# kofinandi/pixel-nerf-yolo

Hardware: NVIDIA B200
Metric: rays/sec (samples/sec) 3-view render at 1/2/4/8 B200 vs host-CPU ref (higher is better)
Workload: dtype bf16

## Files before the change

### pixel-nerf-yolo_b200/csrc/mlp_umma_pair.cu

```cuda
#include "pnr_common.cuh"
#include "umma.cuh"
#include <cuda.h>
#include <stdlib.h>
#include <vector>

namespace pnr {
using namespace umma;

namespace pair {

#ifdef PNR_DIAG_MMAONLY
#define PNR_DIAG_OFF_RING
#define PNR_DIAG_OFF_WAITS
#define PNR_DIAG_OFF_EPI
#define PNR_DIAG_OFF_GATHER
#endif
#ifdef PNR_DIAG_NORING
#define PNR_DIAG_OFF_RING
#define PNR_DIAG_OFF_EMPTY_COMMIT
#endif

constexpr int kNCol = 64;
constexpr int kMT = 2;
constexpr int kKBlocksH = kHidden / kBlockK;
#ifndef PNR_STAGES
#define PNR_STAGES 5
#endif
constexpr int kStages = PNR_STAGES;
constexpr int kThreads = 512;
constexpr int kProducers = 3;
constexpr int kGatherWarps = 4;
constexpr int kEpiWarps = 8;
constexpr int kOperandKB = kNCol * kRowBytes;
constexpr int kChunkBytes = 2 * kOperandKB;
constexpr int kTmemCols = 512;
constexpr int kHCol = 256;
constexpr int kMaxStages = 1024;

struct Sched { int n_blocks, CL, n_linz, KBz, order, proj; };
enum { MAT_LIN_IN = 0, MAT_LINZ = 1, MAT_FC0 = 2, MAT_FC1 = 3, MAT_LIN_OUT = 4 };
struct Seg { int kind, blk, t, len; };
struct StageSrc { int mat, blk, row0, k0; };

__host__ __device__ inline int z_passes(const Sched& s) { return (s.KBz + 7) / 8; }
__host__ __device__ inline int sched_total(const Sched& s) {
  return kMT + s.n_linz * kMT * s.KBz + s.n_blocks * 32 + kKBlocksH;
}
__host__ __device__ inline int sched_pre(const Sched& s) { return kMT + s.n_linz * kMT * s.KBz + s.CL * 32; }
__host__ __device__ inline void fc_pair(int order, int t, int& kc, int& mt, int& kk, bool& first, bool& last) {
  const int pr = t >> 1;
  kk = t & 1;
  if (order == 0) {
    kc = pr >> 1; mt = pr & 1;
    first = pr < 2 && kk == 0; last = pr >= 6 && kk == 1;
    return;
  }
  if (order == 3) {
    kc = (int)((0x23023101u >> (4 * pr)) & 0xFu);
    mt = (int)((0xE4u >> pr) & 1u);
    first = (pr == 0 || pr == 2) && kk == 0;
    last = (pr == 4 || pr == 7) && kk == 1;
    return;
  }
  kc = (pr < 4) ? (pr & 1) : (2 + (pr & 1));
  if (order == 2) kc ^= 1;
  mt = (pr >> 1) & 1;
  first = (pr == 0 || pr == 2) && kk == 0;
  last = (pr == 5 || pr == 7) && kk == 1;
}
__host__ __device__ inline int out_chunk(int order, int t) { return order >= 2 ? ((t >> 1) ^ 1) : (t >> 1); }
__host__ __device__ inline Seg walk_stage(const Sched& sc, int s) {
  Seg g;
  const int s1 = kMT * sc.KBz;
  if (s < kMT) { g.kind = MAT_LIN_IN; g.blk = 0; g.t = s; g.len = kMT; return g; }
  s -= kMT;
  if (s < s1) { g.kind = MAT_LINZ; g.blk = 0; g.t = s; g.len = s1; return g; }
  s -= s1;
  for (int b = 0; b < sc.n_blocks; ++b) {
    const bool has_z = b + 1 < sc.n_linz;
    if (s < 16) { g.kind = MAT_FC0; g.blk = b; g.t = s; g.len = 16; return g; }
    s -= 16;
    if (has_z) {
      if (s < s1) { g.kind = MAT_LINZ; g.blk = b + 1; g.t = s; g.len = s1; return g; }
      s -= s1;
    }
    if (s < 16) { g.kind = MAT_FC1; g.blk = b; g.t = s; g.len = 16; return g; }
    s -= 16;
  }
  g.kind = MAT_LIN_OUT; g.blk = 0; g.t = s; g.len = kKBlocksH;
  return g;
}
struct ZPos { int pass, mt, kbi, kp; };
__host__ __device__ inline ZPos z_position(int KBz, int t) {
  ZPos z;
  z.pass = t / (kMT * 8);
  const int tt = t - z.pass * kMT * 8;
  z.kp = KBz - z.pass * 8 < 8 ? KBz - z.pass * 8 : 8;
  z.mt = tt / z.kp;
  z.kbi = tt - z.mt * z.kp;
  return z;
}
__host__ __device__ inline StageSrc decode_stage(const Sched& sc, int s) {
  const Seg g = walk_stage(sc, s);
  StageSrc r;
  r.mat = g.kind; r.blk = g.blk;
  switch (g.kind) {
    case MAT_LIN_IN: r.row0 = g.t * 256; r.k0 = 0; break;
    case MAT_LINZ: { const ZPos z = z_position(sc.KBz, g.t); r.row0 = z.mt * 256; r.k0 = (z.pass * 8 + z.kbi) * 64; } break;
    case MAT_FC0:
    case MAT_FC1: { int kc, mt, kk; bool f, l; fc_pair(sc.order, g.t, kc, mt, kk, f, l); r.row0 = mt * 256; r.k0 = kc * 128 + kk * 64; } break;
    default: r.row0 = 0; r.k0 = out_chunk(sc.order, g.t) * 128 + (g.t & 1) * 64; break;
  }
  return r;
}

__global__ void pack_stages_kernel(pnr_mlp_params mp, Sched sc, uint8_t* __restrict__ stages) {
  const int s = blockIdx.x >> 1, half = blockIdx.x & 1;
  const StageSrc src = decode_stage(sc, s);
  const float* W; int rows, cols;
  switch (src.mat) {
    case MAT_LIN_IN: W = mp.lin_in_w; rows = mp.d_hidden; cols = mp.d_in; break;
    case MAT_LINZ: W = mp.linz_w[src.blk]; rows = mp.d_hidden; cols = mp.d_latent; break;
    case MAT_FC0: W = mp.fc0_w[src.blk]; rows = mp.d_hidden; cols = mp.d_hidden; break;
    case MAT_FC1: W = mp.fc1_w[src.blk]; rows = mp.d_hidden; cols = mp.d_hidden; break;
    default: W = mp.lin_out_w; rows = mp.d_out; cols = mp.d_hidden; break;
  }
  const bool identity = sc.proj && src.mat == MAT_LINZ;
  uint8_t* dst = stages + ((size_t)s * 2 + half) * kStageBytes;
  for (int i = threadIdx.x; i < kStageRows * kBlockK; i += blockDim.x) {
    const int r = i / kBlockK, k = i % kBlockK;
    const int gr = src.row0 + half * 128 + r, gk = src.k0 + k;
    const float v = identity ? (gr == gk ? 1.f : 0.f) : ((gr < rows && gk < cols) ? W[(size_t)gr * cols + gk] : 0.f);
    *reinterpret_cast<__nv_bfloat16*>(dst + swz_offset(r, k)) = __float2bfloat16_rn(v);
  }
}

struct Smem {
  static constexpr uint32_t w = 0;
  static constexpr uint32_t ring = w + kStages * kStageBytes;
  static constexpr uint32_t lat = ring + 4 * kChunkBytes;
  static constexpr uint32_t zf = lat + kKBlocksH * kOperandKB;
  static constexpr uint32_t bars = zf + kOperandKB;
  static constexpr uint32_t prog = bars + 512;
  static constexpr uint32_t total = prog + 8 * kMaxStages;
};
enum {
  B_W_FULL = 0, B_W_EMPTY = B_W_FULL + kStages, B_IN_READY = B_W_EMPTY + kStages, B_IN_FREE,
  B_X_FULL, B_H_FULL = B_X_FULL + kMT,
  B_RDY = B_H_FULL + kMT, B_X_FREE = B_RDY + 4,
  B_LAND = B_X_FREE + kMT,
  B_OUT_FREE = B_LAND + kMT,
  B_C0_FREE,
  B_COUNT
};
static_assert(B_COUNT <= 30, "barrier parity bits live in one 32-bit word");
static_assert(Smem::total <= 227 * 1024, "shared memory budget");

struct ProgEntry { uint32_t w0, w1; };
__device__ inline ProgEntry make_prog(const Sched& sc, int s, uint32_t sbase) {
  const Seg g = walk_stage(sc, s);
  uint32_t b_addr = 0, dcol = 0, acc = 1, wait_id = 0, c1 = 0, c2 = 0, c3 = 0;
  const bool last = g.t == g.len - 1;
  switch (g.kind) {
    case MAT_LIN_IN:
      b_addr = sbase + Smem::zf; dcol = g.t * 128; acc = 0;
      if (g.t == 0) wait_id = B_IN_READY + 1;
      break;
    case MAT_LINZ: {
      const ZPos z = z_position(sc.KBz, g.t);
      const bool streaming = z_passes(sc) > 1 || sc.proj;
      const bool pass_first = z.mt == 0 && z.kbi == 0, pass_last = z.mt == kMT - 1 && z.kbi == z.kp - 1;
      b_addr = sbase + Smem::lat + z.kbi * kOperandKB; dcol = z.mt * 128;
      if (streaming && pass_first && !(g.blk == 0 && z.pass == 0)) wait_id = B_IN_READY + 1;
      if (pass_last && (streaming || g.blk == sc.n_linz - 1)) c1 = B_IN_FREE + 1;
      if (last && g.blk == 0) { c2 = B_X_FULL + 1; c3 = B_X_FULL + 2; }
    } break;
    case MAT_FC0:
    case MAT_FC1: {
      int kc, mt, kk;
      bool first_of_tile, last_of_tile;
      fc_pair(sc.order, g.t, kc, mt, kk, first_of_tile, last_of_tile);
      const bool fc0 = g.kind == MAT_FC0;
      b_addr = sbase + Smem::ring + (kc * 2 + kk) * kOperandKB; dcol = (fc0 ? kHCol : 0) + mt * 128;
      if (fc0) acc = first_of_tile ? 0 : 1;
      if (mt == 0 && kk == 0) wait_id = B_RDY + kc + 1;
      if (last_of_tile) c2 = (fc0 ? B_H_FULL : B_X_FULL) + mt + 1;
      if (sc.order == 3 && g.t == 11) c1 = B_C0_FREE + 1;
    } break;
    default: {
      const int kc = out_chunk(sc.order, g.t), kk = g.t % 2;
      b_addr = sbase + Smem::ring + (kc * 2 + kk) * kOperandKB; dcol = kHCol; acc = g.t > 0;
      if (kk == 0) wait_id = B_RDY + kc + 1;
      if (last) c2 = B_H_FULL + 1;
    } break;
  }
  ProgEntry e;
  e.w0 = ((b_addr >> 4) & 0x3FFFu) | (dcol << 14) | (acc << 23) | (wait_id << 25);
  e.w1 = c1 | (c2 << 5) | (c3 << 14) | ((c1 | c2 | c3) ? (1u << 19) : 0u);
  return e;
}

__device__ __forceinline__ int gather_col(int gw, int i) { return gw + kGatherWarps * i; }

__device__ __forceinline__ uint32_t pack_relu_bf16x2(float lo, float hi) {
  uint32_t d;
  asm("cvt.rn.relu.bf16x2.f32 %0, %1, %2;" : "=r"(d) : "f"(hi), "f"(lo));
  return d;
}

template <int NC, bool REMOTE, bool ADD_BIAS>
__device__ __forceinline__ void store_transposed(uint32_t base, const uint32_t* vals, float bias, int lane, int kq, int row0,
                                                 uint32_t async_bar = 0) {
  const int g = lane >> 3, i = lane & 7;
  const int k = kq + 8 * g;
  const uint32_t kb_off = (uint32_t)(k >> 6) * kOperandKB;
#pragma unroll
  for (int c0 = 0; c0 < NC; c0 += 16) {
    uint32_t p[8];
#ifdef PNR_DIAG_EPI_NOALU
#pragma unroll
    for (int j = 0; j < 8; ++j) p[j] = (uint32_t)(lane + j + c0);
#else
#pragma unroll
    for (int j = 0; j < 8; ++j) {
      float x = __uint_as_float(vals[c0 + j]), y = __uint_as_float(vals[c0 + 8 + j]);
      if (ADD_BIAS) { x += bias; y += bias; }
      p[j] = pack_relu_bf16x2(x, y);
    }
    transpose8x8(p, lane);
#endif
    const uint32_t e0 = __byte_perm(p[0], p[1], 0x5410), e1 = __byte_perm(p[2], p[3], 0x5410);
// ... 32 lines not shown
  const int pair_id = blockIdx.x >> 1, n_pairs = gridDim.x >> 1;
  constexpr int PP = kNCol / NS;
  constexpr int G = kNCol / PP;
  constexpr int NLIVE = G * PP;
  const bool pooled = NS > 1 || sch.CL < sch.n_blocks;
  const int n_sg = ((n_tiles + 1) / 2 + G - 1) / G;
  float* const xbar = xbar_all + (size_t)pair_id * (2 * kNCol * kHidden);
  extern __shared__ __align__(1024) uint8_t smem[];
  const uint32_t sbase = smem_u32(smem);
  volatile uint32_t* tmem_base_slot = reinterpret_cast<volatile uint32_t*>(smem + Smem::bars + 8 * B_COUNT);
  const int warp = __shfl_sync(0xffffffffu, (int)(threadIdx.x >> 5), 0);
  const int lane = threadIdx.x & 31;
  long long* const prof = (PROF == 1 && g_prof_pair) ? reinterpret_cast<long long*>(smem + Smem::bars + 256) : nullptr;
  if (prof && threadIdx.x < 32) prof[threadIdx.x] = 0;
  long long* const trace = (PROF == 2 && g_trace_pair && (blockIdx.x >> 1) == 0) ? g_trace_pair : nullptr;
  int n_tr = 0;
  const bool trace_stages = PROF == 2 && trace && g_trace_stages;
  auto bar = [&](int i) -> uint32_t { return sbase + Smem::bars + 8u * i; };
  auto lbar = [&](int i) -> uint32_t { return mapa_u32(sbase + Smem::bars + 8u * i, 0); };
  if ((sbase & 1023u) != 0) { if (threadIdx.x == 0) printf("pnr: dynamic smem not 1024-aligned\n"); __trap(); }

  if (threadIdx.x == 0) {
    for (int i = 0; i < kStages; ++i) { mbar_init(bar(B_W_FULL + i), 1); mbar_init(bar(B_W_EMPTY + i), 1); }
    mbar_init(bar(B_IN_READY), 2 * kGatherWarps);
    mbar_init(bar(B_IN_FREE), 1);
    for (int i = 0; i < kMT; ++i) { mbar_init(bar(B_X_FULL + i), 1); mbar_init(bar(B_H_FULL + i), 1); }
    for (int i = 0; i < 4; ++i) mbar_init(bar(B_RDY + i), kEpiWarps + ((ASYNC && (i & 1) == 0) ? 1 : 0));
    for (int i = 0; i < kMT; ++i) mbar_init(bar(B_LAND + i), kEpiWarps);
    mbar_init(bar(B_OUT_FREE), 2);
    mbar_init(bar(B_C0_FREE), 1);
    for (int i = 0; i < kMT; ++i) mbar_init(bar(B_X_FREE + i), 2 * kEpiWarps);
    fence_barrier_init();
  }
  const int n_stages = sched_total(sch);
  const int s_pre = sched_pre(sch);
  const int n_flat = G * s_pre + (n_stages - s_pre);
  for (int i = threadIdx.x; i < n_stages; i += kThreads) {
    const ProgEntry pe = make_prog(sch, i, sbase);
    reinterpret_cast<ProgEntry*>(smem + Smem::prog)[i] = pe;
    if (i == n_stages - 1) reinterpret_cast<ProgEntry*>(smem + Smem::prog)[n_stages] = pe;
  }
  if (warp == 1) tmem_alloc_2sm(sbase + Smem::bars + 8 * B_COUNT, kTmemCols);
  tc_fence_before();
  __syncthreads();
  cluster_sync_all();
  tc_fence_after();
  const uint32_t tmem_base = __shfl_sync(0xffffffffu, *tmem_base_slot, 0);
  if (warp == 4) PTRACE_L0(1 + (int)crank, 0xFF);
#ifdef PNR_DIAG_N
  const uint32_t idesc = instr_desc_bf16_2sm(PNR_DIAG_N);
#else
  const uint32_t idesc = instr_desc_bf16_2sm(2 * kNCol);
#endif

  if (warp == 0 || warp == 12 || warp == 13) {
    const int pid = warp == 0 ? 0 : warp - 11;
    if (elect_one()) {
      uint32_t slot = pid, par = 1;
      int carry = pid;
      for (int sg = pair_id; sg < n_sg; sg += n_pairs) {
        int fi = carry;
        int st = fi < G * s_pre ? fi % s_pre : fi - (G - 1) * s_pre;
        for (; fi < n_flat; fi += kProducers) {
#ifdef PNR_DIAG_OFF_RING
          continue;
#endif
          PTRACE(5 + pid + 3 * (int)crank, 0x10 + B_W_EMPTY + slot);
#if PNR_IDLE_WAIT
          mbar_wait_idle(bar(B_W_EMPTY + slot), par);
#else
          mbar_wait_cluster(bar(B_W_EMPTY + slot), par);
#endif
          PTRACE(5 + pid + 3 * (int)crank, 0x40 + B_W_EMPTY + slot);
#ifdef PNR_DIAG_NOWEIGHTS
          if (crank == 0) mbar_arrive(bar(B_W_FULL + slot));
#else
          if (crank == 0) mbar_arrive_expect_tx(bar(B_W_FULL + slot), 2 * kStageBytes);
          tma_load_2d_2sm(sbase + Smem::w + slot * kStageBytes, &wmap, 0, (st * 2 + (int)crank) * kStageRows, bar(B_W_FULL + slot));
#endif
          PTRACE(5 + pid + 3 * (int)crank, 0x84);
          slot += kProducers;
          if (slot >= kStages) { slot -= kStages; par ^= 1; }
          const int nf = fi + kProducers;
          if (nf < G * s_pre) { st += kProducers; if (st >= s_pre) st -= s_pre; }
          else st = nf - (G - 1) * s_pre;
        }
        carry = fi - n_flat;
      }
    }
    __syncwarp();
  } else if (warp == 1) {
    if (crank == 0) {
      const long long t_role0 = prof ? clock64() : 0;
      if (elect_one()) {
        uint32_t slot = 0, wpar = 0, ph = 0;
        uint32_t full_bar = bar(B_W_FULL), empty_bar = bar(B_W_EMPTY);
        const uint64_t wdesc0 = smem_desc(sbase + Smem::w);
        uint64_t a_desc = wdesc0;
        const uint64_t bdesc_hi = smem_desc(0);
        constexpr uint64_t kStageStep = kStageBytes >> 4;
        const uint2* prog = reinterpret_cast<const uint2*>(smem + Smem::prog);
#define MPROF_T0() const long long t0__ = prof ? clock64() : 0
#define MPROF_ADD(slot_) do { if (prof) prof[slot_] += clock64() - t0__; } while (0)
        for (int sg = pair_id; sg < n_sg; sg += n_pairs) {
          for (int seg = 0; seg <= G; ++seg) {
            const bool after_mean = seg > 0 && seg < G;
            if (after_mean) {
              MPROF_T0();
#ifndef PNR_DIAG_OFF_WAITS
              mbar_wait_cluster(bar(B_X_FREE), (ph >> B_X_FREE) & 1u);
#endif
              ph ^= (1u << B_X_FREE);
              tc_fence_after();
              MPROF_ADD(5);
            }
            const int st_beg = seg < G ? 0 : s_pre, st_end = seg < G ? s_pre : n_stages;
            if (seg == 0 && sg != pair_id) {
#ifndef PNR_DIAG_OFF_WAITS
              mbar_wait(bar(B_OUT_FREE), (ph >> B_OUT_FREE) & 1u);
#endif
              ph ^= (1u << B_OUT_FREE);
            }
            uint2 cur = prog[st_beg];
            auto issue_stage = [&](int st) {
              const uint2 nxt = prog[st + 1];
              const uint32_t wait_id = cur.x >> 25;
              if (wait_id) {
                MPROF_T0();
                const uint32_t id = wait_id - 1;
                PTRACE(0, 0x10 + id);
#ifndef PNR_DIAG_OFF_WAITS
                mbar_wait_cluster(bar(id), (ph >> id) & 1u);
#endif
                ph ^= (1u << id);
                PTRACE(0, 0x40 + id);
                if (ASYNC) fence_proxy_async();
                tc_fence_after();
                MPROF_ADD(id == B_IN_READY ? 2 : 4);
              }
#ifndef PNR_DIAG_OFF_RING
              {
                MPROF_T0();
                mbar_wait(full_bar, wpar);
                MPROF_ADD(1);
                if (trace_stages) PTRACE(0, 0x72);
              }
#endif
              const uint64_t b_desc = bdesc_hi | (uint64_t)(cur.x & 0x3FFFu);
              const uint32_t d_col = (cur.x >> 14) & 0x1FFu;
              mma_kblock_desc_2sm(tmem_base + d_col, a_desc, b_desc, idesc, (cur.x >> 23) & 1u);
#ifndef PNR_DIAG_OFF_EMPTY_COMMIT
              mma_commit_2sm(empty_bar, 3);
#endif
              if (cur.y & (1u << 19)) {
                const uint32_t c1 = cur.y & 31u, c2 = (cur.y >> 5) & 31u, c3 = (cur.y >> 14) & 31u;
                if (c1) mma_commit_2sm(bar(c1 - 1), 3);
                if (c2) mma_commit_2sm(bar(c2 - 1), 3);
                if (c3) mma_commit_2sm(bar(c3 - 1), 3);
                if (PROF == 2 && c2 > B_X_FULL && c2 <= B_X_FULL + 4) PTRACE(0, c2 - B_X_FULL);
              }
              if (trace_stages) PTRACE(0, 0x71);
              if (++slot == kStages) { slot = 0; wpar ^= 1; full_bar = bar(B_W_FULL); empty_bar = bar(B_W_EMPTY); a_desc = wdesc0; }
              else { full_bar += 8; empty_bar += 8; a_desc += kStageStep; }
              cur = nxt;
            };
            int st = st_beg;
            if (after_mean) {
              issue_stage(st++);
              MPROF_T0();
#ifndef PNR_DIAG_OFF_WAITS
              mbar_wait_cluster(bar(B_X_FREE + 1), (ph >> (B_X_FREE + 1)) & 1u);
#endif
              ph ^= (1u << (B_X_FREE + 1));
              tc_fence_after();
              MPROF_ADD(5);
            }
            for (; st < st_end; ++st) issue_stage(st);
          }
        }
#undef MPROF_T0
#undef MPROF_ADD
      }
      __syncwarp();
      if (prof && lane == 0) prof[0] += clock64() - t_role0;
#ifdef PNR_DIAG_OFF_EPI
    } else if (false) {
#else
    } else if (ASYNC) {
#endif
      const int n_pub = G * 2 * sch.CL + 2 * (sch.n_blocks - sch.CL) + 1;
      uint32_t par = 0;
      for (int sg = pair_id; sg < n_sg; sg += n_pairs) {
        for (int i = 0; i < n_pub; ++i) {
#pragma unroll
          for (int mt = 0; mt < kMT; ++mt) {
            mbar_wait_cluster(bar(B_LAND + mt), par);
// ... 273 lines not shown
              const uint4* src = reinterpret_cast<const uint4*>(fl0 + vb + off);
              r[2 * k] = __ldg(src); r[2 * k + 1] = __ldg(src + 1);
            } else {
              r[2 * k] = make_uint4(0u, 0u, 0u, 0u); r[2 * k + 1] = make_uint4(0u, 0u, 0u, 0u);
            }
          }
        };
        auto blend_col = [&](int i, const uint4 (&r)[8], const float (&w)[4]) {
          if (!act) return;
          float acc[16];
#pragma unroll
          for (int j = 0; j < 16; ++j) acc[j] = 0.f;
#pragma unroll
          for (int k = 0; k < 4; ++k) {
            const __nv_bfloat162* h0 = reinterpret_cast<const __nv_bfloat162*>(&r[2 * k]);
            const __nv_bfloat162* h1 = reinterpret_cast<const __nv_bfloat162*>(&r[2 * k + 1]);
#pragma unroll
            for (int j = 0; j < 4; ++j) {
              const float2 f0 = __bfloat1622float2(h0[j]), f1 = __bfloat1622float2(h1[j]);
              acc[2 * j] += w[k] * f0.x; acc[2 * j + 1] += w[k] * f0.y;
              acc[8 + 2 * j] += w[k] * f1.x; acc[8 + 2 * j + 1] += w[k] * f1.y;
            }
          }
          uint4 o0, o1;
          __nv_bfloat162* q0 = reinterpret_cast<__nv_bfloat162*>(&o0);
          __nv_bfloat162* q1 = reinterpret_cast<__nv_bfloat162*>(&o1);
#pragma unroll
          for (int j = 0; j < 4; ++j) {
            q0[j] = __floats2bfloat162_rn(acc[2 * j], acc[2 * j + 1]);
            q1[j] = __floats2bfloat162_rn(acc[8 + 2 * j], acc[8 + 2 * j + 1]);
          }
          const int c = gather_col(gw, i);
          uint8_t* kb_base = smem + Smem::lat + (lane >> 2) * kOperandKB;
          const int k_in = (lane & 3) * 16;
          *reinterpret_cast<uint4*>(kb_base + swz_offset(c, k_in)) = o0;
          *reinterpret_cast<uint4*>(kb_base + swz_offset(c, k_in + 8)) = o1;
        };
        {
          uint4 ra[8], rb[8];
          float wa[4], wb[4];
          load_col(0, ra, wa);
          load_col(1, rb, wb);
          {
            PPROF_T0();
            if (gw == 0 && crank == 0) PTRACE_L0(4, 0x10 + B_IN_FREE);
#if PNR_IDLE_WAIT
            mbar_wait_idle(bar(B_IN_FREE), par_free);
#else
            mbar_wait_cluster(bar(B_IN_FREE), par_free);
#endif
            if (gw == 0 && crank == 0) PTRACE_L0(4, 0x40 + B_IN_FREE);
            if (gw == 0) PPROF_ADD(17);
          }
          par_free ^= 1;
          if (fill == 0) {
#pragma unroll 1
            for (int i = 0; i < 16; ++i) zfeat_col(i);
          }
#pragma unroll 1
          for (int i = 0; i < 16; i += 2) {
            blend_col(i, ra, wa);
            if (i + 2 < 16) load_col(i + 2, ra, wa);
            blend_col(i + 1, rb, wb);
            if (i + 3 < 16) load_col(i + 3, rb, wb);
          }
        }
        fence_proxy_async();
        __syncwarp();
        if (lane == 0) { if (crank == 0) mbar_arrive(bar(B_IN_READY)); else mbar_arrive_cluster_relaxed(lbar(B_IN_READY)); }
        if (gw == 0 && crank == 0) PTRACE_L0(4, 0x83);
      }
    }
    if (prof && gw == 0 && lane == 0) prof[16] += clock64() - t_role0;
  }

  tc_fence_before();
  __syncthreads();
  if (PROF == 1 && g_prof_pair && threadIdx.x < 32) g_prof_pair[(size_t)blockIdx.x * 32 + threadIdx.x] = prof[threadIdx.x];
  cluster_sync_all();
  if (warp == 1) tmem_dealloc_2sm(tmem_base, kTmemCols);
}

}

static bool pair_async() {
  static int cached = -1;
  if (cached < 0) { const char* e = getenv("PNR_ASYNC"); cached = (e && atoi(e) == 0) ? 0 : 1; }
  return cached != 0;
}
static int pair_order() {
  static int cached = -1;
  if (cached < 0) { const char* e = getenv("PNR_ORDER"); cached = e ? atoi(e) : 2; if (cached < 0 || cached > 3) cached = 2; }
  return cached;
}
static pair::Sched pair_sched(const pnr_mlp_params* p, int proj) {
  return pair::Sched{p->n_blocks, p->combine_layer, p->combine_layer, proj ? kHidden / 64 : p->d_latent / 64, pair_order(), proj};
}
size_t pair_stream_bytes(const pnr_mlp_params* p, int proj) {
  pair::Sched s = pair_sched(p, proj);
  return (size_t)pair::sched_total(s) * 2 * kStageBytes;
}
int pair_stages(const pnr_mlp_params* p, int proj) {
  pair::Sched s = pair_sched(p, proj);
  return pair::sched_total(s);
}
int pair_pack(const pnr_mlp_params* p, uint8_t* stream, int proj, cudaStream_t st) {
  pair::Sched s = pair_sched(p, proj);
  PNR_REQUIRE(pair::sched_total(s) < pair::kMaxStages, PNR_ERR_UNSUPPORTED, "pair_pack: %d stages exceed the stage program (one padding entry is needed)", pair::sched_total(s));
  pair::pack_stages_kernel<<<pair::sched_total(s) * 2, 256, 0, st>>>(*p, s, stream);
  PNR_CHECK_LAUNCH("pair::pack_stages_kernel");
  return PNR_OK;
}

size_t pair_workspace_bytes() {
  int dev = 0, sms = 148;
  cudaGetDevice(&dev);
  cudaDeviceGetAttribute(&sms, cudaDevAttrMultiProcessorCount, dev);
  return (size_t)(sms / 2) * 2 * pair::kNCol * kHidden * sizeof(float);
}

int field_forward_pair(const pnr_scene* sc, const pnr_points* q, const pnr_mlp_params* mp, const uint8_t* stream,
                       const float* bx, const float* bh, const float* bo, float* out, void* ws, size_t ws_bytes,
                       int num_freqs, float freq_factor, int raw, int proj, cudaStream_t st) {
  PNR_REQUIRE(ws && ws_bytes >= pair_workspace_bytes() && ((uintptr_t)ws & 15) == 0, PNR_ERR_ARG,
              "field_forward_pair: workspace of pnr_field_workspace_bytes() = %zu bytes required (got %zu)",
              pair_workspace_bytes(), ws_bytes);
  float* xbar = (float*)ws;
  pair::Sched sch = pair_sched(mp, proj);
  const int PP = pair::kNCol / sc->NS;
  const int tiles_per_obj = (q->P + PP - 1) / PP;
  const long long n_tiles_ll = (long long)tiles_per_obj * sc->SB;
  PNR_REQUIRE(n_tiles_ll < (1LL << 31), PNR_ERR_ARG, "field_forward_pair: too many tiles");
  const int n_tiles = (int)n_tiles_ll;
  typedef CUresult (*EncodeFn)(CUtensorMap*, CUtensorMapDataType, cuuint32_t, void*, const cuuint64_t*, const cuuint64_t*,
                               const cuuint32_t*, const cuuint32_t*, CUtensorMapInterleave, CUtensorMapSwizzle,
                               CUtensorMapL2promotion, CUtensorMapFloatOOBfill);
  static EncodeFn encode = nullptr;
  if (!encode) {
    void* fn = nullptr;
    cudaDriverEntryPointQueryResult qres;
    cudaError_t e = cudaGetDriverEntryPoint("cuTensorMapEncodeTiled", &fn, cudaEnableDefault, &qres);
    PNR_REQUIRE(e == cudaSuccess && fn, PNR_ERR_CUDA, "cuTensorMapEncodeTiled entry point not found");
    encode = (EncodeFn)fn;
  }
  CUtensorMap tmap;
  cuuint64_t gdim[2] = {64, (cuuint64_t)pair::sched_total(sch) * 256};
  cuuint64_t gstride[1] = {128};
  cuuint32_t box[2] = {64, 128};
  cuuint32_t estr[2] = {1, 1};
  CUresult r = encode(&tmap, CU_TENSOR_MAP_DATA_TYPE_BFLOAT16, 2, (void*)stream, gdim, gstride, box, estr,
                      CU_TENSOR_MAP_INTERLEAVE_NONE, CU_TENSOR_MAP_SWIZZLE_NONE, CU_TENSOR_MAP_L2_PROMOTION_L2_256B,
                      CU_TENSOR_MAP_FLOAT_OOB_FILL_NONE);
  PNR_REQUIRE(r == CUDA_SUCCESS, PNR_ERR_CUDA, "cuTensorMapEncodeTiled failed (%d)", (int)r);
  int dev = 0, sms = 148;
  cudaGetDevice(&dev);
  cudaDeviceGetAttribute(&sms, cudaDevAttrMultiProcessorCount, dev);
  const int G = pair::kNCol / PP;
  const bool async_x = pair_async();
  const bool vmax = mp->combine_type == PNR_COMBINE_MAX && sc->NS > 1;
  PNR_REQUIRE(!vmax || (async_x && !getenv("PNR_TRACE") && !getenv("PNR_PROF")), PNR_ERR_UNSUPPORTED,
              "field_forward_pair: the PNR_ASYNC=0 / PNR_PROF / PNR_TRACE instruments are built for combine_type average only");
  const int n_groups = ((n_tiles + 1) / 2 + G - 1) / G;
  long long* prof_dev = nullptr;
  long long* trace_dev = nullptr;
  if (getenv("PNR_TRACE")) {
    cudaMalloc(&trace_dev, (size_t)11 * pair::kTraceLen * sizeof(long long));
    cudaMemset(trace_dev, 0, (size_t)11 * pair::kTraceLen * sizeof(long long));
    cudaMemcpyToSymbol(pair::g_trace_pair, &trace_dev, sizeof(trace_dev));
    const int ts = getenv("PNR_TRACE_STAGES") ? 1 : 0;
    cudaMemcpyToSymbol(pair::g_trace_stages, &ts, sizeof(ts));
  } else if (getenv("PNR_PROF")) {
    cudaMalloc(&prof_dev, (size_t)4096 * 32 * sizeof(long long));
    cudaMemset(prof_dev, 0, (size_t)4096 * 32 * sizeof(long long));
    cudaMemcpyToSymbol(pair::g_prof_pair, &prof_dev, sizeof(prof_dev));
  }
#define PNR_LAUNCH_PAIR(NSV)                                                                                     \
  case NSV: {                                                                                                    \
    auto kern = vmax ? pair::field_pair_kernel<NSV, true, 0, (NSV > 1)>                                          \
              : async_x ? (trace_dev ? pair::field_pair_kernel<NSV, true, 2> : prof_dev ? pair::field_pair_kernel<NSV, true, 1> : pair::field_pair_kernel<NSV, true, 0>) \
// ... 66 lines not shown
```

### pixel-nerf-yolo_b200/csrc/umma.cuh

```cuda
#pragma once
#include <cuda_runtime.h>
#include <cuda_bf16.h>
#include <stdint.h>

namespace pnr {
namespace umma {

constexpr int kBlockK = 64;
constexpr int kRowBytes = 128;
constexpr int kUmmaK = 16;
constexpr int kStageRows = 128;
constexpr int kStageBytes = kStageRows * kRowBytes;

__host__ __device__ __forceinline__ uint32_t swz_offset(int row, int k) {
  return (uint32_t)(row * kRowBytes + ((((k >> 3) ^ (row & 7)) & 7) << 4) + ((k & 7) << 1));
}

__device__ __forceinline__ uint32_t smem_u32(const void* p) {
  return (uint32_t)__cvta_generic_to_shared(p);
}

__device__ __forceinline__ uint32_t elect_one() {
  uint32_t pred;
  asm volatile(
// ... 103 lines not shown
  asm volatile(
      "cp.async.bulk.shared::cluster.global.mbarrier::complete_tx::bytes.multicast::cluster [%0], [%1], %2, [%3], %4;" ::"r"(
          dst_smem),
      "l"(src), "r"(bytes), "r"(bar), "h"(cta_mask)
      : "memory");
}

__device__ __forceinline__ uint32_t cluster_ctarank() {
  uint32_t r;
  asm volatile("mov.u32 %0, %%cluster_ctarank;" : "=r"(r));
  return r;
}
__device__ __forceinline__ uint32_t cluster_nctarank() {
  uint32_t r;
  asm volatile("mov.u32 %0, %%cluster_nctarank;" : "=r"(r));
  return r;
}
__device__ __forceinline__ void cluster_sync_all() {
  asm volatile("barrier.cluster.arrive.release.aligned;" ::: "memory");
  asm volatile("barrier.cluster.wait.acquire.aligned;" ::: "memory");
}

__device__ __forceinline__ void tmem_alloc(uint32_t dst_smem, uint32_t ncols) {
  asm volatile("tcgen05.alloc.cta_group::1.sync.aligned.shared::cta.b32 [%0], %1;" ::"r"(dst_smem), "r"(ncols) : "memory");
  asm volatile("tcgen05.relinquish_alloc_permit.cta_group::1.sync.aligned;" ::: "memory");
}
__device__ __forceinline__ void tmem_dealloc(uint32_t taddr, uint32_t ncols) {
  asm volatile("tcgen05.dealloc.cta_group::1.sync.aligned.b32 %0, %1;" ::"r"(taddr), "r"(ncols) : "memory");
}

__device__ __forceinline__ uint64_t smem_desc(uint32_t saddr) {
  return (uint64_t)((saddr >> 4) & 0x3FFFu) | (1ull << 16) | (64ull << 32) | (1ull << 46) | (2ull << 61);
}
__host__ __device__ __forceinline__ uint32_t instr_desc_bf16(int n) {
  return (1u << 4) | (1u << 7) | (1u << 10) | ((uint32_t)(n >> 3) << 17) | ((uint32_t)(128 >> 4) << 24);
}

__device__ __forceinline__ void mma_bf16(uint32_t d_tmem, uint64_t a_desc, uint64_t b_desc, uint32_t idesc,
                                         uint32_t accumulate) {
  asm volatile(
      "{\n\t.reg .pred p;\n\t"
      "setp.ne.b32 p, %4, 0;\n\t"
      "tcgen05.mma.cta_group::1.kind::f16 [%0], %1, %2, %3, p;\n\t}" ::"r"(d_tmem),
      "l"(a_desc), "l"(b_desc), "r"(idesc), "r"(accumulate)
      : "memory");
}
__device__ __forceinline__ void mma_commit(uint32_t bar) {
  asm volatile("tcgen05.commit.cta_group::1.mbarrier::arrive::one.shared::cluster.b64 [%0];" ::"r"(bar) : "memory");
}

__device__ __forceinline__ void mma_commit_multicast(uint32_t bar, uint16_t cta_mask) {
  asm volatile("tcgen05.commit.cta_group::1.mbarrier::arrive::one.shared::cluster.multicast::cluster.b64 [%0], %1;" ::"r"(bar),
               "h"(cta_mask)
               : "memory");
}

__device__ __forceinline__ void mma_kblock_desc(uint32_t d_tmem, uint64_t a_desc, uint64_t b_desc, uint32_t idesc,
                                                bool accumulate_first) {
#pragma unroll
  for (int ks = 0; ks < kBlockK / kUmmaK; ++ks)
    mma_bf16(d_tmem, a_desc + 2 * ks, b_desc + 2 * ks, idesc, (accumulate_first || ks > 0) ? 1u : 0u);
}

__device__ __forceinline__ void mma_kblock(uint32_t d_tmem, uint32_t a_base, uint32_t b_base, uint32_t idesc,
                                           bool accumulate_first) {
#pragma unroll
// ... 160 lines not shown
```

### pixel-nerf-yolo_b200/model/models.py

```python
import os
import os.path as osp
import warnings

import torch

from .. import _lib
from .code import PositionalEncoding
from .model_util import make_encoder, make_mlp


class _FieldTrainFn(torch.autograd.Function):

    @staticmethod
    def forward(ctx, net, mlp, mode, sb, feat, a, b, *params):
        lib = _lib.load()
        dev = feat.device
        sc, keep = net._scene_for(feat, fp32_maps=True)
        pts = _lib.points_rays(a, b, sb) if mode == "rays" else _lib.points_xyz(a, b)
        P = pts.P
        cp = mlp.c_params()
        out = torch.empty(sb, P, net.d_out, device=dev, dtype=torch.float32)
        tape = torch.empty(lib.pnr_field_tape_bytes(sc, pts, cp), dtype=torch.uint8, device=dev)
        with torch.cuda.device(dev):
            rc = lib.pnr_field_forward_train(sc, pts, cp, out.data_ptr(), tape.data_ptr(), tape.numel(),
# ... 149 lines not shown
        NS = self.num_views_per_obj
        self._check_views()
        SB = n_views // NS
        dev = self.poses.device
        if self._cam_cache is None:
            def per_view(t):
                t = t.to(dev).float()
                if t.shape[0] == 1:
                    return t.expand(n_views, 2).contiguous()
                if t.shape[0] == SB:
                    return t.unsqueeze(1).expand(SB, NS, 2).reshape(n_views, 2).contiguous()
                if t.shape[0] == n_views:
                    return t.contiguous()
                raise AssertionError(f"focal/c has {t.shape[0]} rows for {SB} objects x {NS} views")
            focal_k = -self.focal if self.yolo else self.focal
            self._cam_cache = (self.poses.contiguous(), per_view(focal_k), per_view(self.c),
                               float(self.image_shape[0]), float(self.image_shape[1]),
                               float(self.encoder.latent_scaling[0]), float(self.encoder.latent_scaling[1]))
        poses, focal, center, iw, ih, lsx, lsy = cams if cams is not None else self._cam_cache
        assert feat.shape[0] == n_views, "encoder.latent and poses disagree on the number of views"
        sc = _lib.Scene()
        sc.feat, sc.poses, sc.focal, sc.center = feat.data_ptr(), poses.data_ptr(), focal.data_ptr(), center.data_ptr()
        sc.SB, sc.NS, sc.C, sc.Hl, sc.Wl = SB, NS, feat.shape[3], feat.shape[1], feat.shape[2]
        sc.feat_fp32 = int(fp32_maps)
        sc.flags = (_lib.SCENE_MASK_NONNEG_Z | _lib.SCENE_RAW_OUTPUT) if self.yolo else 0
        if fp32_maps and self.train_precision == "tf32":
            sc.flags |= _lib.SCENE_TRAIN_TF32
        elif fp32_maps and self.train_precision == "bf16":
            sc.flags |= _lib.SCENE_TRAIN_BF16
        sc.image_w, sc.image_h, sc.lat_scale_x, sc.lat_scale_y = iw, ih, lsx, lsy
        return sc, (poses, focal, center, iw, ih, lsx, lsy)

    def projects_latent(self) -> bool:
        proj = self.project_wide_latent
        if proj is None:
            proj = self.mlp_coarse.d_latent > self.mlp_coarse.d_hidden
        return bool(proj)

    def _scene_bf16(self, mlp, proj: bool):
        if proj:
            feat = mlp.project_features(self.encoder.packed_latent(fp32=True), self.encoder.generation)
            sc, keep = self._scene_for(feat, fp32_maps=False)
            sc.flags |= _lib.SCENE_PROJECTED
            return sc, (keep, feat)
        return self._scene(fp32_maps=False)

    def render_scenes(self):
        proj = self.projects_latent()
        sc_c, keep_c = self._scene_bf16(self.mlp_coarse, proj)
        if proj and self.mlp_fine is not None:
            sc_f, keep_f = self._scene_bf16(self.mlp_fine, proj)
            return sc_c, sc_f, (keep_c, keep_f)
        return sc_c, None, (keep_c,)

    def render_state_key(self):
        mf = self.mlp_fine
        return (self.encoder.generation, self._cam_gen, self.num_views_per_obj, self.projects_latent(), self.precision,
                self.mlp_coarse._param_key(), None if mf is None else mf._param_key())

    def _mlp(self, coarse):
        return self.mlp_coarse if (coarse or self.mlp_fine is None) else self.mlp_fine

    def _run_field(self, pts: "_lib.Points", SB: int, P: int, coarse: bool, keep) -> torch.Tensor:
        dev = self.poses.device
        _lib.require_device(dev)
        lib = _lib.load()
        mlp = self._mlp(coarse)
        out = torch.empty(SB, P, self.d_out, device=dev, dtype=torch.float32)
        if P == 0:
            return out
# ... 120 lines not shown
```

Baseline: 390,700.

## Synthesize identity weights in shared memory for projected-latent linz stages

When latent features are pre-projected, the linz stages multiply by an identity matrix. These stages are no longer streamed through the weight ring: the MMA warp now uses a small identity operand built once in shared memory and interleaves these MMAs with fc1 tiles. This removes weight-ring traffic and waits for those stages and shortens the packed weight stream. It also makes projection the default path and repacks the gather layout to match. The cost is more complex schedule bookkeeping, a new non-swizzled descriptor path, and a tighter shared-memory stage-program budget.

```diff
diff --git a/pixel-nerf-yolo_b200/csrc/mlp_umma_pair.cu b/pixel-nerf-yolo_b200/csrc/mlp_umma_pair.cu
--- a/pixel-nerf-yolo_b200/csrc/mlp_umma_pair.cu
+++ b/pixel-nerf-yolo_b200/csrc/mlp_umma_pair.cu
@@ -35,18 +35,22 @@
 constexpr int kChunkBytes = 2 * kOperandKB;
 constexpr int kTmemCols = 512;
 constexpr int kHCol = 256;
-constexpr int kMaxStages = 1024;
 
 struct Sched { int n_blocks, CL, n_linz, KBz, order, proj; };
 enum { MAT_LIN_IN = 0, MAT_LINZ = 1, MAT_FC0 = 2, MAT_FC1 = 3, MAT_LIN_OUT = 4 };
 struct Seg { int kind, blk, t, len; };
 struct StageSrc { int mat, blk, row0, k0; };
 
+constexpr int kIdentStages = 8;
+
 __host__ __device__ inline int z_passes(const Sched& s) { return (s.KBz + 7) / 8; }
-__host__ __device__ inline int sched_total(const Sched& s) {
-  return kMT + s.n_linz * kMT * s.KBz + s.n_blocks * 32 + kKBlocksH;
-}
-__host__ __device__ inline int sched_pre(const Sched& s) { return kMT + s.n_linz * kMT * s.KBz + s.CL * 32; }
+__host__ __device__ inline int linz_len(const Sched& s, bool stream) {
+  return s.proj ? (stream ? 0 : kIdentStages) : kMT * s.KBz;
+}
+__host__ __device__ inline int sched_total(const Sched& s, bool stream) {
+  return kMT + s.n_linz * linz_len(s, stream) + s.n_blocks * 32 + kKBlocksH;
+}
+__host__ __device__ inline int sched_pre(const Sched& s, bool stream) { return kMT + s.n_linz * linz_len(s, stream) + s.CL * 32; }
 __host__ __device__ inline void fc_pair(int order, int t, int& kc, int& mt, int& kk, bool& first, bool& last) {
   const int pr = t >> 1;
   kk = t & 1;
@@ -68,10 +72,18 @@
   first = (pr == 0 || pr == 2) && kk == 0;
   last = (pr == 5 || pr == 7) && kk == 1;
 }
+__host__ __device__ inline int fc1_tile0_last(int order) {
+  for (int t = 0; t < 16; ++t) {
+    int kc, mt, kk; bool f, l;
+    fc_pair(order, t, kc, mt, kk, f, l);
+    if (l && mt == 0) return t;
+  }
+  return 15;
+}
 __host__ __device__ inline int out_chunk(int order, int t) { return order >= 2 ? ((t >> 1) ^ 1) : (t >> 1); }
-__host__ __device__ inline Seg walk_stage(const Sched& sc, int s) {
+__host__ __device__ inline Seg walk_stage(const Sched& sc, int s, bool stream) {
   Seg g;
-  const int s1 = kMT * sc.KBz;
+  const int s1 = linz_len(sc, stream);
   if (s < kMT) { g.kind = MAT_LIN_IN; g.blk = 0; g.t = s; g.len = kMT; return g; }
   s -= kMT;
   if (s < s1) { g.kind = MAT_LINZ; g.blk = 0; g.t = s; g.len = s1; return g; }
@@ -80,6 +92,18 @@
     const bool has_z = b + 1 < sc.n_linz;
     if (s < 16) { g.kind = MAT_FC0; g.blk = b; g.t = s; g.len = 16; return g; }
     s -= 16;
+    if (has_z && sc.proj && !stream) {
+      if (s < 24) {
+        const int l0 = fc1_tile0_last(sc.order);
+        if (s <= l0) { g.kind = MAT_FC1; g.blk = b; g.t = s; g.len = 16; }
+        else if (s <= l0 + 4) { g.kind = MAT_LINZ; g.blk = b + 1; g.t = s - l0 - 1; g.len = kIdentStages; }
+        else if (s < 20) { g.kind = MAT_FC1; g.blk = b; g.t = s - 4; g.len = 16; }
+        else { g.kind = MAT_LINZ; g.blk = b + 1; g.t = s - 16; g.len = kIdentStages; }
+        return g;
+      }
+      s -= 24;
+      continue;
+    }
     if (has_z) {
       if (s < s1) { g.kind = MAT_LINZ; g.blk = b + 1; g.t = s; g.len = s1; return g; }
       s -= s1;
@@ -101,7 +125,7 @@
   return z;
 }
 __host__ __device__ inline StageSrc decode_stage(const Sched& sc, int s) {
-  const Seg g = walk_stage(sc, s);
+  const Seg g = walk_stage(sc, s, true);
   StageSrc r;
   r.mat = g.kind; r.blk = g.blk;
   switch (g.kind) {
@@ -125,25 +149,28 @@
     case MAT_FC1: W = mp.fc1_w[src.blk]; rows = mp.d_hidden; cols = mp.d_hidden; break;
     default: W = mp.lin_out_w; rows = mp.d_out; cols = mp.d_hidden; break;
   }
-  const bool identity = sc.proj && src.mat == MAT_LINZ;
   uint8_t* dst = stages + ((size_t)s * 2 + half) * kStageBytes;
   for (int i = threadIdx.x; i < kStageRows * kBlockK; i += blockDim.x) {
     const int r = i / kBlockK, k = i % kBlockK;
     const int gr = src.row0 + half * 128 + r, gk = src.k0 + k;
-    const float v = identity ? (gr == gk ? 1.f : 0.f) : ((gr < rows && gk < cols) ? W[(size_t)gr * cols + gk] : 0.f);
+    const float v = (gr < rows && gk < cols) ? W[(size_t)gr * cols + gk] : 0.f;
     *reinterpret_cast<__nv_bfloat16*>(dst + swz_offset(r, k)) = __float2bfloat16_rn(v);
   }
 }
 
+constexpr int kIdentCores = 47;
+__host__ __device__ constexpr int ident_core(int c) { return c == 0 ? 15 : 31; }
 struct Smem {
   static constexpr uint32_t w = 0;
   static constexpr uint32_t ring = w + kStages * kStageBytes;
   static constexpr uint32_t lat = ring + 4 * kChunkBytes;
   static constexpr uint32_t zf = lat + kKBlocksH * kOperandKB;
-  static constexpr uint32_t bars = zf + kOperandKB;
+  static constexpr uint32_t ident = zf + kOperandKB;
+  static constexpr uint32_t bars = ident + ((kIdentCores * 128 + 1023) & ~1023);
   static constexpr uint32_t prog = bars + 512;
-  static constexpr uint32_t total = prog + 8 * kMaxStages;
+  static constexpr uint32_t total = 227 * 1024;
 };
+constexpr int kMaxStages = (Smem::total - Smem::prog) / 8;
 enum {
   B_W_FULL = 0, B_W_EMPTY = B_W_FULL + kStages, B_IN_READY = B_W_EMPTY + kStages, B_IN_FREE,
   B_X_FULL, B_H_FULL = B_X_FULL + kMT,
@@ -154,27 +181,39 @@
   B_COUNT
 };
 static_assert(B_COUNT <= 30, "barrier parity bits live in one 32-bit word");
-static_assert(Smem::total <= 227 * 1024, "shared memory budget");
+static_assert(kMaxStages > 8 * (kMT * 8 + 32) + kMT + kKBlocksH, "stage program: every schedule with d_latent <= 512 must fit");
+static_assert(kStages != 5 || (Smem::ident == 216 * 1024 && Smem::bars == 222 * 1024 && kMaxStages == 576),
+              "shared memory map (5-slot ring): 80 + 64 + 64 + 8 KiB operands, 6 KiB identity, 512 B barriers, 4.5 KiB program");
 
 struct ProgEntry { uint32_t w0, w1; };
 __device__ inline ProgEntry make_prog(const Sched& sc, int s, uint32_t sbase) {
-  const Seg g = walk_stage(sc, s);
-  uint32_t b_addr = 0, dcol = 0, acc = 1, wait_id = 0, c1 = 0, c2 = 0, c3 = 0;
+  const Seg g = walk_stage(sc, s, false);
+  uint32_t b_addr = 0, dcol = 0, acc = 1, wait_id = 0, c1 = 0, c2 = 0, c3 = 0, ident = 0;
   const bool last = g.t == g.len - 1;
   switch (g.kind) {
     case MAT_LIN_IN:
       b_addr = sbase + Smem::zf; dcol = g.t * 128; acc = 0;
       if (g.t == 0) wait_id = B_IN_READY + 1;
       break;
-    case MAT_LINZ: {
-      const ZPos z = z_position(sc.KBz, g.t);
-      const bool streaming = z_passes(sc) > 1 || sc.proj;
-      const bool pass_first = z.mt == 0 && z.kbi == 0, pass_last = z.mt == kMT - 1 && z.kbi == z.kp - 1;
-      b_addr = sbase + Smem::lat + z.kbi * kOperandKB; dcol = z.mt * 128;
-      if (streaming && pass_first && !(g.blk == 0 && z.pass == 0)) wait_id = B_IN_READY + 1;
-      if (pass_last && (streaming || g.blk == sc.n_linz - 1)) c1 = B_IN_FREE + 1;
-      if (last && g.blk == 0) { c2 = B_X_FULL + 1; c3 = B_X_FULL + 2; }
-    } break;
+    case MAT_LINZ:
+      if (sc.proj) {
+        const int mt = g.t >> 2, c = (g.t >> 1) & 1, h = g.t & 1;
+        b_addr = sbase + Smem::lat + (4 * mt + 2 * c + h) * kOperandKB; dcol = mt * 128;
+        ident = (uint32_t)(ident_core(c) - 8 * h);
+        if (g.t == 0 && g.blk > 0) wait_id = B_IN_READY + 1;
+        if (last) c1 = B_IN_FREE + 1;
+        if (g.blk == 0) { if (last) { c2 = B_X_FULL + 1; c3 = B_X_FULL + 2; } }
+        else if ((g.t & 3) == 3) c2 = B_X_FULL + mt + 1;
+      } else {
+        const ZPos z = z_position(sc.KBz, g.t);
+        const bool streaming = z_passes(sc) > 1;
+        const bool pass_first = z.mt == 0 && z.kbi == 0, pass_last = z.mt == kMT - 1 && z.kbi == z.kp - 1;
+        b_addr = sbase + Smem::lat + z.kbi * kOperandKB; dcol = z.mt * 128;
+        if (streaming && pass_first && !(g.blk == 0 && z.pass == 0)) wait_id = B_IN_READY + 1;
+        if (pass_last && (streaming || g.blk == sc.n_linz - 1)) c1 = B_IN_FREE + 1;
+        if (last && g.blk == 0) { c2 = B_X_FULL + 1; c3 = B_X_FULL + 2; }
+      }
+      break;
     case MAT_FC0:
     case MAT_FC1: {
       int kc, mt, kk;
@@ -184,7 +223,8 @@
       b_addr = sbase + Smem::ring + (kc * 2 + kk) * kOperandKB; dcol = (fc0 ? kHCol : 0) + mt * 128;
       if (fc0) acc = first_of_tile ? 0 : 1;
       if (mt == 0 && kk == 0) wait_id = B_RDY + kc + 1;
-      if (last_of_tile) c2 = (fc0 ? B_H_FULL : B_X_FULL) + mt + 1;
+      const bool z_follows = !fc0 && sc.proj && g.blk + 1 < sc.n_linz;
+      if (last_of_tile && !z_follows) c2 = (fc0 ? B_H_FULL : B_X_FULL) + mt + 1;
       if (sc.order == 3 && g.t == 11) c1 = B_C0_FREE + 1;
     } break;
     default: {
@@ -196,7 +236,7 @@
   }
   ProgEntry e;
   e.w0 = ((b_addr >> 4) & 0x3FFFu) | (dcol << 14) | (acc << 23) | (wait_id << 25);
-  e.w1 = c1 | (c2 << 5) | (c3 << 14) | ((c1 | c2 | c3) ? (1u << 19) : 0u);
+  e.w1 = c1 | (c2 << 5) | (c3 << 14) | ((c1 | c2 | c3) ? (1u << 19) : 0u) | (ident << 20);
   return e;
 }
 
@@ -295,13 +335,20 @@
     for (int i = 0; i < kMT; ++i) mbar_init(bar(B_X_FREE + i), 2 * kEpiWarps);
     fence_barrier_init();
   }
-  const int n_stages = sched_total(sch);
-  const int s_pre = sched_pre(sch);
-  const int n_flat = G * s_pre + (n_stages - s_pre);
+  const int n_stages = sched_total(sch, false);
+  const int s_pre = sched_pre(sch, false);
   for (int i = threadIdx.x; i < n_stages; i += kThreads) {
     const ProgEntry pe = make_prog(sch, i, sbase);
     reinterpret_cast<ProgEntry*>(smem + Smem::prog)[i] = pe;
     if (i == n_stages - 1) reinterpret_cast<ProgEntry*>(smem + Smem::prog)[n_stages] = pe;
+  }
+  if (sch.proj) {
+    uint32_t* id = reinterpret_cast<uint32_t*>(smem + Smem::ident);
+    for (int i = threadIdx.x; i < kIdentCores * 32; i += kThreads) {
+      const int core = i >> 5, row = (i >> 2) & 7, pair = i & 3;
+      id[i] = (core == ident_core((int)crank) && (row >> 1) == pair) ? (0x3F80u << (16 * (row & 1))) : 0u;
+    }
+    fence_proxy_async();
   }
   if (warp == 1) tmem_alloc_2sm(sbase + Smem::bars + 8 * B_COUNT, kTmemCols);
   tc_fence_before();
@@ -318,12 +365,14 @@
 
   if (warp == 0 || warp == 12 || warp == 13) {
     const int pid = warp == 0 ? 0 : warp - 11;
+    const int w_pre = sched_pre(sch, true);
+    const int n_flat = G * w_pre + (sched_total(sch, true) - w_pre);
     if (elect_one()) {
       uint32_t slot = pid, par = 1;
       int carry = pid;
       for (int sg = pair_id; sg < n_sg; sg += n_pairs) {
         int fi = carry;
-        int st = fi < G * s_pre ? fi % s_pre : fi - (G - 1) * s_pre;
+        int st = fi < G * w_pre ? fi % w_pre : fi - (G - 1) * w_pre;
         for (; fi < n_flat; fi += kProducers) {
 #ifdef PNR_DIAG_OFF_RING
           continue;
@@ -345,8 +394,8 @@
           slot += kProducers;
           if (slot >= kStages) { slot -= kStages; par ^= 1; }
           const int nf = fi + kProducers;
-          if (nf < G * s_pre) { st += kProducers; if (st >= s_pre) st -= s_pre; }
-          else st = nf - (G - 1) * s_pre;
+          if (nf < G * w_pre) { st += kProducers; if (st >= w_pre) st -= w_pre; }
+          else st = nf - (G - 1) * w_pre;
         }
         carry = fi - n_flat;
       }
@@ -361,6 +410,7 @@
         const uint64_t wdesc0 = smem_desc(sbase + Smem::w);
         uint64_t a_desc = wdesc0;
         const uint64_t bdesc_hi = smem_desc(0);
+        const uint64_t idesc_m1 = smem_desc_interleave(sbase + Smem::ident - 128, 128, 128);
         constexpr uint64_t kStageStep = kStageBytes >> 4;
         const uint2* prog = reinterpret_cast<const uint2*>(smem + Smem::prog);
 #define MPROF_T0() const long long t0__ = prof ? clock64() : 0
@@ -401,20 +451,30 @@
                 tc_fence_after();
                 MPROF_ADD(id == B_IN_READY ? 2 : 4);
               }
-#ifndef PNR_DIAG_OFF_RING
-              {
-                MPROF_T0();
-                mbar_wait(full_bar, wpar);
-                MPROF_ADD(1);
-                if (trace_stages) PTRACE(0, 0x72);
-              }
-#endif
               const uint64_t b_desc = bdesc_hi | (uint64_t)(cur.x & 0x3FFFu);
               const uint32_t d_col = (cur.x >> 14) & 0x1FFu;
-              mma_kblock_desc_2sm(tmem_base + d_col, a_desc, b_desc, idesc, (cur.x >> 23) & 1u);
+              const uint32_t ident = cur.y >> 20;
+              if (ident) {
+                const uint64_t a_id = idesc_m1 + ((uint64_t)ident << 3);
+#pragma unroll
+                for (int ks = 0; ks < kBlockK / kUmmaK; ++ks)
+                  mma_bf16_2sm(tmem_base + d_col, a_id - 16 * ks, b_desc + 2 * ks, idesc, 1u);
+              } else {
+#ifndef PNR_DIAG_OFF_RING
+                {
+                  MPROF_T0();
+                  mbar_wait(full_bar, wpar);
+                  MPROF_ADD(1);
+                  if (trace_stages) PTRACE(0, 0x72);
+                }
+#endif
+                mma_kblock_desc_2sm(tmem_base + d_col, a_desc, b_desc, idesc, (cur.x >> 23) & 1u);
 #ifndef PNR_DIAG_OFF_EMPTY_COMMIT
-              mma_commit_2sm(empty_bar, 3);
-#endif
+                mma_commit_2sm(empty_bar, 3);
+#endif
+                if (++slot == kStages) { slot = 0; wpar ^= 1; full_bar = bar(B_W_FULL); empty_bar = bar(B_W_EMPTY); a_desc = wdesc0; }
+                else { full_bar += 8; empty_bar += 8; a_desc += kStageStep; }
+              }
               if (cur.y & (1u << 19)) {
                 const uint32_t c1 = cur.y & 31u, c2 = (cur.y >> 5) & 31u, c3 = (cur.y >> 14) & 31u;
                 if (c1) mma_commit_2sm(bar(c1 - 1), 3);
@@ -423,8 +483,6 @@
                 if (PROF == 2 && c2 > B_X_FULL && c2 <= B_X_FULL + 4) PTRACE(0, c2 - B_X_FULL);
               }
               if (trace_stages) PTRACE(0, 0x71);
-              if (++slot == kStages) { slot = 0; wpar ^= 1; full_bar = bar(B_W_FULL); empty_bar = bar(B_W_EMPTY); a_desc = wdesc0; }
-              else { full_bar += 8; empty_bar += 8; a_desc += kStageStep; }
               cur = nxt;
             };
             int st = st_beg;
@@ -764,9 +822,9 @@
           }
           const int c = gather_col(gw, i);
           uint8_t* kb_base = smem + Smem::lat + (lane >> 2) * kOperandKB;
-          const int k_in = (lane & 3) * 16;
-          *reinterpret_cast<uint4*>(kb_base + swz_offset(c, k_in)) = o0;
-          *reinterpret_cast<uint4*>(kb_base + swz_offset(c, k_in + 8)) = o1;
+          const int k_in = (lane & 3) * 16, sw = sch.proj ? 8 : 0;
+          *reinterpret_cast<uint4*>(kb_base + swz_offset(c, k_in + sw)) = o0;
+          *reinterpret_cast<uint4*>(kb_base + swz_offset(c, k_in + 8 - sw)) = o1;
         };
         {
           uint4 ra[8], rb[8];
@@ -830,16 +888,23 @@
 }
 size_t pair_stream_bytes(const pnr_mlp_params* p, int proj) {
   pair::Sched s = pair_sched(p, proj);
-  return (size_t)pair::sched_total(s) * 2 * kStageBytes;
+  return (size_t)pair::sched_total(s, true) * 2 * kStageBytes;
 }
 int pair_stages(const pnr_mlp_params* p, int proj) {
   pair::Sched s = pair_sched(p, proj);
-  return pair::sched_total(s);
+  return pair::sched_total(s, true);
+}
+static int check_program(const pair::Sched& s, const char* who) {
+  PNR_REQUIRE(pair::sched_total(s, false) < pair::kMaxStages, PNR_ERR_UNSUPPORTED,
+              "%s: %d stages exceed the %d-entry stage program (one padding entry is needed); fewer blocks before combine_layer or "
+              "pre-projected maps (PNR_SCENE_PROJECTED) shorten it", who, pair::sched_total(s, false), pair::kMaxStages);
+  return PNR_OK;
 }
 int pair_pack(const pnr_mlp_params* p, uint8_t* stream, int proj, cudaStream_t st) {
   pair::Sched s = pair_sched(p, proj);
-  PNR_REQUIRE(pair::sched_total(s) < pair::kMaxStages, PNR_ERR_UNSUPPORTED, "pair_pack: %d stages exceed the stage program (one padding entry is needed)", pair::sched_total(s));
-  pair::pack_stages_kernel<<<pair::sched_total(s) * 2, 256, 0, st>>>(*p, s, stream);
+  const int rc = check_program(s, "pair_pack");
+  if (rc) return rc;
+  pair::pack_stages_kernel<<<pair::sched_total(s, true) * 2, 256, 0, st>>>(*p, s, stream);
   PNR_CHECK_LAUNCH("pair::pack_stages_kernel");
   return PNR_OK;
 }
@@ -859,6 +924,8 @@
               pair_workspace_bytes(), ws_bytes);
   float* xbar = (float*)ws;
   pair::Sched sch = pair_sched(mp, proj);
+  const int rc = check_program(sch, "field_forward_pair");
+  if (rc) return rc;
   const int PP = pair::kNCol / sc->NS;
   const int tiles_per_obj = (q->P + PP - 1) / PP;
   const long long n_tiles_ll = (long long)tiles_per_obj * sc->SB;
@@ -876,7 +943,7 @@
     encode = (EncodeFn)fn;
   }
   CUtensorMap tmap;
-  cuuint64_t gdim[2] = {64, (cuuint64_t)pair::sched_total(sch) * 256};
+  cuuint64_t gdim[2] = {64, (cuuint64_t)pair::sched_total(sch, true) * 256};
   cuuint64_t gstride[1] = {128};
   cuuint32_t box[2] = {64, 128};
   cuuint32_t estr[2] = {1, 1};
diff --git a/pixel-nerf-yolo_b200/csrc/umma.cuh b/pixel-nerf-yolo_b200/csrc/umma.cuh
--- a/pixel-nerf-yolo_b200/csrc/umma.cuh
+++ b/pixel-nerf-yolo_b200/csrc/umma.cuh
@@ -159,6 +159,9 @@
 __device__ __forceinline__ uint64_t smem_desc(uint32_t saddr) {
   return (uint64_t)((saddr >> 4) & 0x3FFFu) | (1ull << 16) | (64ull << 32) | (1ull << 46) | (2ull << 61);
 }
+__device__ __forceinline__ uint64_t smem_desc_interleave(uint32_t saddr, uint32_t lbo, uint32_t sbo) {
+  return (uint64_t)((saddr >> 4) & 0x3FFFu) | ((uint64_t)(lbo >> 4) << 16) | ((uint64_t)(sbo >> 4) << 32) | (1ull << 46);
+}
 __host__ __device__ __forceinline__ uint32_t instr_desc_bf16(int n) {
   return (1u << 4) | (1u << 7) | (1u << 10) | ((uint32_t)(n >> 3) << 17) | ((uint32_t)(128 >> 4) << 24);
 }
diff --git a/pixel-nerf-yolo_b200/model/models.py b/pixel-nerf-yolo_b200/model/models.py
--- a/pixel-nerf-yolo_b200/model/models.py
+++ b/pixel-nerf-yolo_b200/model/models.py
@@ -205,10 +205,7 @@
         return sc, (poses, focal, center, iw, ih, lsx, lsy)
 
     def projects_latent(self) -> bool:
-        proj = self.project_wide_latent
-        if proj is None:
-            proj = self.mlp_coarse.d_latent > self.mlp_coarse.d_hidden
-        return bool(proj)
+        return self.project_wide_latent is None or bool(self.project_wide_latent)
 
     def _scene_bf16(self, mlp, proj: bool):
         if proj:
```

New measurement: 328,500 (median of 6 runs). -15.9%, worse.
